# timlawrenz/DINO-X

Measured on AMD Instinct MI355X. Metric: training images/sec (source samples; 2 global views each) ViT-S/16 224px bs256/GPU, higher is better.
Workload: dtype bf16; 1 GPU; ViT-S/16 224x224x3 2.5D slice stacks, scale-aware, 2 views/sample, DINO+Gram loss, AdamW+EMA; per_gpu_batch=256, global_batch=256, local_crops=0, out_dim=8192, parallelism=dp1, hipgraph=False

## Files before the change

### dino-x_amd/csrc/gemm_bf16_areg.hip

```cpp
#include "common.h"
#include "kernels.h"
#include <type_traits>

namespace dinox {

typedef __attribute__((address_space(3))) void ar_lds_void;
typedef __attribute__((address_space(1))) const void ar_gbl_void;
typedef unsigned ar_u32x4 __attribute__((ext_vector_type(4)));

typedef float ar_f32x4 __attribute__((ext_vector_type(4)));

template <bool NT, typename V>
__device__ __forceinline__ void ar_store(char* dst, V v) {
  if (NT) __builtin_nontemporal_store(v, reinterpret_cast<V*>(dst));
  else *reinterpret_cast<V*>(dst) = v;
}

constexpr int AR_BK = 32, AR_BM = 128, AR_BN = 128;
constexpr int AR_SETS = 6;
constexpr int AR_ATILE = AR_BM * AR_BK * 2, AR_BTILE = AR_BN * AR_BK * 2, AR_SLOT = AR_ATILE + AR_BTILE;
constexpr int AR_KBLOCK = 6 * AR_BK * 2;

enum { AR_PLAIN = EPI_ACT_PLAIN, AR_GELU = EPI_ACT_GELU, AR_DGELU = EPI_ACT_DGELU };

__device__ __forceinline__ int ar_xcd_remap(int bid, int nwg) {
  const int q = nwg >> 3, r = nwg & 7, xcd = bid & 7, idx = bid >> 3;
  return (xcd < r ? xcd * (q + 1) : r * (q + 1) + (xcd - r) * q) + idx;
}

template <int OUT_DT, int ACT, bool RES, bool NT>
__global__ __launch_bounds__(256, 3) void gemm_bf16_nt_areg(GemmParams p, int ntiles, int tiles_n) {
  extern __shared__ __attribute__((aligned(16))) char smem[];
  const int lane = threadIdx.x & 63;
  const int wv = __builtin_amdgcn_readfirstlane(threadIdx.x >> 6);
  const int wr = wv >> 1, wc = wv & 1;
  const int tile = ar_xcd_remap(blockIdx.x, ntiles);
  const int tm = tile / tiles_n, tn = tile - tm * tiles_n;
  const int64_t m0 = (int64_t)tm * AR_BM, n0 = (int64_t)tn * AR_BN;
// ... 236 lines not shown
            }
          } else {
#pragma unroll
            for (int u = 0; u < 4; ++u) {
              a[u] = v[u];
              v[u] = gelu_fast(v[u]);
            }
          }
          if (OUT_DT == DINOX_BF16) {
            pa[2 * h] = (unsigned)f32_to_bf16(a[0]) | ((unsigned)f32_to_bf16(a[1]) << 16);
            pa[2 * h + 1] = (unsigned)f32_to_bf16(a[2]) | ((unsigned)f32_to_bf16(a[3]) << 16);
          } else if (p.aux) {
            ar_store<NT>(ablk + ai + 16 * h, ar_f32x4{a[0], a[1], a[2], a[3]});
          }
        }
        if (ACT == AR_DGELU) {
          float x[4];
          if (OUT_DT == DINOX_BF16) {
            const float4 raw = cur_aux[it][0];
            const unsigned w0 = __float_as_uint(h ? raw.z : raw.x), w1 = __float_as_uint(h ? raw.w : raw.y);
            x[0] = __uint_as_float(w0 << 16); x[1] = __uint_as_float(w0 & 0xffff0000u);
            x[2] = __uint_as_float(w1 << 16); x[3] = __uint_as_float(w1 & 0xffff0000u);
          } else {
            const float4 xv = cur_aux[it][h ? AUXV - 1 : 0];
            x[0] = xv.x; x[1] = xv.y; x[2] = xv.z; x[3] = xv.w;
          }
          if (ag) {
#pragma unroll
            for (int u = 0; u < 4; ++u) v[u] *= x[u];
          } else {
// ... 62 lines not shown
```

### dino-x_amd/csrc/gemm_bf16_glds.hip

```cpp

#include "small_common.h"
#include "kernels.h"

namespace dinox {

constexpr int GG_BN = 128;

typedef __attribute__((address_space(3))) void lds_void;
typedef __attribute__((address_space(1))) const void gbl_void;

__device__ __forceinline__ int gg_xcd_remap(int bid, int nwg) {
  const int q = nwg >> 3, r = nwg & 7, xcd = bid & 7, idx = bid >> 3;
  return (xcd < r ? xcd * (q + 1) : r * (q + 1) + (xcd - r) * q) + idx;
}

enum { GG_PLAIN = 0, GG_GELU = 1, GG_DGELU = 2 };

template <int CH>
__device__ __forceinline__ int gg_swz(int row) { return CH == 8 ? ((row >> 1) & 7) : ((row >> 2) & 3); }

template <int OUT_DT, int ACT, bool RES, int GG_BK, int STAGES, int GG_BM>
__global__ __launch_bounds__(256, (GG_BM == 256 ? 2 : (GG_BK == 64 ? 2 : 3))) void gemm_bf16_nt_glds(GemmParams p, int tiles_m, int tiles_n) {
  constexpr int WAVES = 4;
  constexpr int WM = GG_BM / 64;
  constexpr int WROWS = 32 * WM;
  constexpr int A_TILE = GG_BM * GG_BK * 2;
  constexpr int B_TILE = GG_BN * GG_BK * 2;
  constexpr int STAGE_BYTES = A_TILE + B_TILE;
  constexpr int CH = GG_BK / 8;
  constexpr int RPI = 64 / CH;
  constexpr int NQA = GG_BM / RPI / WAVES;
// ... 199 lines not shown
          }
        }
        if (p.aux) {
          const int64_t ai = bz * p.M * p.ldaux + m * p.ldaux + n;
          if (OUT_DT == DINOX_BF16) {
            s16x8 pk;
#pragma unroll
            for (int u = 0; u < 8; ++u) pk[u] = (short)f32_to_bf16(a[u]);
            __builtin_nontemporal_store(pk, reinterpret_cast<s16x8*>((bf16_t*)p.aux + ai));
          } else {
            *reinterpret_cast<float4*>((float*)p.aux + ai) = make_float4(a[0], a[1], a[2], a[3]);
            *reinterpret_cast<float4*>((float*)p.aux + ai + 4) = make_float4(a[4], a[5], a[6], a[7]);
          }
        }
      }
      if (ACT == GG_DGELU) {
        float x[8];
        if (OUT_DT == DINOX_BF16) {
          const float4 raw = cur_aux[it][0];
          const uint32_t w[4] = {__float_as_uint(raw.x), __float_as_uint(raw.y), __float_as_uint(raw.z), __float_as_uint(raw.w)};
#pragma unroll
          for (int u = 0; u < 4; ++u) {
            x[2 * u] = __uint_as_float(w[u] << 16);
            x[2 * u + 1] = __uint_as_float(w[u] & 0xffff0000u);
          }
        } else {
          const float4 x0 = cur_aux[it][0], x1 = cur_aux[it][OUT_DT == DINOX_BF16 ? 0 : 1];
          x[0] = x0.x; x[1] = x0.y; x[2] = x0.z; x[3] = x0.w; x[4] = x1.x; x[5] = x1.y; x[6] = x1.z; x[7] = x1.w;
        }
        if (p.epilogue & DINOX_EPI_AUXGRAD) {
// ... 47 lines not shown
  int bk_auto = p.K <= 512 ? 32 : 64;
  if (bk_auto == 64) {
    const int64_t nt = ceil_div(p.M, (int64_t)128) * ceil_div(p.N, (int64_t)GG_BN) * p.batch;
    const double e512 = (double)nt / (double)(ceil_div(nt, (int64_t)512) * 512), e768 = (double)nt / (double)(ceil_div(nt, (int64_t)768) * 768);
    if (0.9 * e768 > e512) bk_auto = 32;
  }
  const int bk = knob ? knob : bk_auto;
  const int bm = knob_bm ? knob_bm : 128;
  const int stages = bk == 64 ? 2 : 3;

  const int tiles_m = (int)ceil_div(p.M, bm), tiles_n = (int)ceil_div(p.N, GG_BN);
  const int64_t ntile = (int64_t)tiles_m * tiles_n;
  if (ntile > 0x7fffffff) return DINOX_EUNSUPPORTED;
  dim3 grid((unsigned)ntile, (unsigned)p.batch);
  const size_t lds = (size_t)stages * (bm + GG_BN) * bk * 2;
  const int act = (p.epilogue & DINOX_EPI_GELU) ? GG_GELU : (p.epilogue & DINOX_EPI_DGELU) ? GG_DGELU : GG_PLAIN;
  const bool res = (p.epilogue & DINOX_EPI_RESIDUAL) != 0;
  auto launch = [&](auto kern) -> int {
    if (int rc = reserve_lds(reinterpret_cast<const void*>(kern), lds, "gemm_bf16_nt_glds")) return rc;
    hipLaunchKernelGGL(kern, grid, dim3(256), lds, st, p, tiles_m, tiles_n);
    return check_launch("gemm_bf16_nt_glds");
  };
#define GG_K(OUT, ACT, RES, BK, ST, BM) launch(gemm_bf16_nt_glds<OUT, ACT, RES, BK, ST, BM>)
#define GG(OUT, ACT, RES)                                                                               \
  (bm == 256 ? (bk == 32 ? GG_K(OUT, ACT, RES, 32, 3, 256) : GG_K(OUT, ACT, RES, 64, 2, 256))           \
             : (bk == 32 ? GG_K(OUT, ACT, RES, 32, 3, 128) : GG_K(OUT, ACT, RES, 64, 2, 128)))
#define GG_ACT(OUT, RES) (act == GG_GELU ? GG(OUT, GG_GELU, RES) : act == GG_DGELU ? GG(OUT, GG_DGELU, RES) : GG(OUT, GG_PLAIN, RES))
  const int rc = p.out_dtype == DINOX_BF16 ? (res ? GG_ACT(DINOX_BF16, true) : GG_ACT(DINOX_BF16, false))
                                           : (res ? GG_ACT(DINOX_F32, true) : GG_ACT(DINOX_F32, false));
#undef GG_ACT
#undef GG
#undef GG_K
  return rc;
}

}
```

### dino-x_amd/csrc/gemm_pp_common.h

```cpp
#pragma once
#include "common.h"
#include "kernels.h"

namespace dinox {

typedef __attribute__((address_space(3))) void pp_lds_void;
typedef __attribute__((address_space(1))) const void pp_gbl_void;
typedef unsigned pp_u32x4 __attribute__((ext_vector_type(4)));
typedef float pp_f32x4 __attribute__((ext_vector_type(4)));
typedef float pp_f32x2 __attribute__((ext_vector_type(2)));
typedef __bf16 pp_bf16x2 __attribute__((ext_vector_type(2)));

enum { PP_PLAIN = EPI_ACT_PLAIN, PP_GELU = EPI_ACT_GELU, PP_DGELU = EPI_ACT_DGELU };

__device__ __forceinline__ unsigned pp_pack2(float a, float b) {
  const pp_bf16x2 r = __builtin_convertvector(pp_f32x2{a, b}, pp_bf16x2);
  return __builtin_bit_cast(unsigned, r);
}

__device__ __forceinline__ void pp_sync() {
  asm volatile("s_waitcnt lgkmcnt(0)" ::: "memory");
  __builtin_amdgcn_s_barrier();
  __builtin_amdgcn_sched_barrier(0);
}

#define PP_WAIT_BEHIND_STORES(BASE, STEP, sq)                                                                             \
  {                                                                                                                       \
    if ((sq) == 0) asm volatile("s_waitcnt vmcnt(%0)" ::"n"(BASE) : "memory");                                            \
// ... 115 lines not shown
      for (int hh = 0; hh < 2; ++hh) {
        __builtin_amdgcn_sched_barrier(0);
        const pp_f32x4 x4 = hh ? hi : lo;
        float v[4] = {x4[0], x4[1], x4[2], x4[3]}, a[4] = {0.f, 0.f, 0.f, 0.f};
#pragma unroll
        for (int e = 0; e < 4; ++e) v[e] = v[e] * alpha + bias[4 * hh + e];
        if (ACT == PP_GELU) {
#pragma unroll
          for (int e = 0; e < 4; ++e) {
            float y, d;
            gelu_fast_both(v[e], y, d);
            a[e] = d;
            v[e] = y;
          }
        }
        if (ACT == PP_DGELU) {
          float x[4];
          if (OUT_DT == DINOX_BF16) {
            const float4 raw = pf_aux[s % NPF][h][0];
            const unsigned w0 = __float_as_uint(hh ? raw.z : raw.x), w1 = __float_as_uint(hh ? raw.w : raw.y);
            x[0] = __uint_as_float(w0 << 16); x[1] = __uint_as_float(w0 & 0xffff0000u);
            x[2] = __uint_as_float(w1 << 16); x[3] = __uint_as_float(w1 & 0xffff0000u);
          } else {
            const float4 xv = pf_aux[s % NPF][h][hh ? AUXV - 1 : 0];
            x[0] = xv.x; x[1] = xv.y; x[2] = xv.z; x[3] = xv.w;
          }
#pragma unroll
          for (int e = 0; e < 4; ++e) v[e] *= x[e];
        }
        if (RES) {
// ... 82 lines not shown
```

### dino-x_amd/csrc/kernels.h

```cpp
#pragma once
#include <type_traits>

#include "gemm_common.h"
#include "knobs.h"

namespace dinox {

#define GEMM_VARIANTS(X)                                                                                                       \
  X(NtPp, "gemm_bf16_nt_pp") X(NtPp128, "gemm_bf16_nt_pp128") X(NtPp384, "gemm_bf16_nt_pp384") X(NtAreg, "gemm_bf16_nt_areg") \
  X(NtGlds, "gemm_bf16_nt_glds") X(Nt, "gemm_bf16_nt") X(TnBig, "gemm_bf16_tn_big") X(TnDma, "gemm_bf16_tn_dma") X(Tn, "gemm_bf16_tn")
#define X(member, name) member,
enum class GemmVariant { None, GEMM_VARIANTS(X) };
#undef X
#define X(member, name) name,
inline const char* gemm_variant_name(GemmVariant v) {
  static const char* const names[] = {nullptr, GEMM_VARIANTS(X)};
  return names[(int)v];
}
#undef X

int launch_gemm_f32(const GemmParams& p, hipStream_t st);
GemmVariant gemm_bf16_variant(const GemmParams& p);
int launch_gemm_bf16(const GemmParams& p, hipStream_t st);
int64_t gemm_bf16_ws_bytes(const GemmParams& p);
// ... 17 lines not shown
int tn_big_plan(const GemmParams& p, int& tiles_m, int& tiles_n, int& splits, int64_t& kps);
int64_t tn_big_ws_bytes(const GemmParams& p);
int launch_gemm_bf16_tn_big(const GemmParams& p, hipStream_t st, int& splits_out, int& tiles_n_out);

int launch_attention_ref_fwd(const void* qkv, void* o, float* lse, int B, int N, int heads, int d, int dtype, hipStream_t st);
int launch_attention_ref_bwd(const void* d_o, const void* qkv, const void* o, const float* lse, void* dqkv, int B, int N, int heads, int d, int dtype, hipStream_t st);
int launch_attention_bf16_fwd(const void* qkv, void* o, float* lse, int B, int N, int heads, int d, hipStream_t st);
int launch_attention_bf16_bwd(const void* d_o, const void* qkv, const void* o, const float* lse, void* dqkv, float* ws, int B, int N, int heads, int d, hipStream_t st);
bool attention_qkv_fused_ok(int B, int N, int heads, int d, int D);
int launch_attention_qkv_fused_fwd(const void* x, const void* w, const float* bias, void* o, void* qkv_out, float* lse, int B, int N, int heads, int d, int D, hipStream_t st);
int launch_attention_flash_fwd(const void* qkv, void* o, float* lse, int B, int N, int heads, int d, hipStream_t st);
int launch_attention_flash_bwd(const void* d_o, const void* qkv, const void* o, const float* lse, void* dqkv, float* ws, int B, int N, int heads, int d, hipStream_t st);

constexpr int SEG_MAX_CLASSES = 64;

enum { EPI_ACT_PLAIN = 0, EPI_ACT_GELU = 1, EPI_ACT_DGELU = 2 };

template <typename F>
static inline int with_epilogue_case(const GemmParams& p, F&& f) {
  const int act = (p.epilogue & DINOX_EPI_GELU) ? EPI_ACT_GELU : (p.epilogue & DINOX_EPI_DGELU) ? EPI_ACT_DGELU : EPI_ACT_PLAIN;
  const bool res = (p.epilogue & DINOX_EPI_RESIDUAL) != 0;
  auto cases = [&](auto out) -> int {
    switch (act * 2 + (res ? 1 : 0)) {
      case 0: return f(out, std::integral_constant<int, EPI_ACT_PLAIN>{}, std::false_type{});
      case 1: return f(out, std::integral_constant<int, EPI_ACT_PLAIN>{}, std::true_type{});
      case 2: return f(out, std::integral_constant<int, EPI_ACT_GELU>{}, std::false_type{});
      case 4: return f(out, std::integral_constant<int, EPI_ACT_DGELU>{}, std::false_type{});
      default: return DINOX_EUNSUPPORTED;
    }
  };
  return p.out_dtype == DINOX_BF16 ? cases(std::integral_constant<int, DINOX_BF16>{}) : cases(std::integral_constant<int, DINOX_F32>{});
}

struct PersistPlan {
  int tiles_n, units, order, stagger;
  unsigned grid;
};
static inline bool persist_plan(const GemmParams& p, int bm, int bn, int stagger_auto, PersistPlan& pl) {
  const int64_t tiles_n = ceil_div(p.N, (int64_t)bn), units = ceil_div(p.M, (int64_t)bm) * tiles_n;
  if (units > 0x3fffffff) return false;
  const int64_t ncu = device_cu_count();
  pl = {(int)tiles_n, (int)units, knob_int("DINOX_PP_ORDER", 1), knob_int("DINOX_PP_STAGGER", stagger_auto), (unsigned)(units < ncu ? units : ncu)};
// ... 5 lines not shown
```

### dino-x_amd/csrc/optim.hip

```cpp
#include "small_common.h"

namespace dinox {

__global__ __launch_bounds__(256) void adamw_ema_kernel(float* __restrict__ p, const float* __restrict__ g, float* __restrict__ m,
                                                        float* __restrict__ v, float* __restrict__ teacher, int64_t n,
                                                        float lr, float wd, float b1, float b2, float eps, float inv_bc1,
                                                        float inv_sqrt_bc2, float ema, float gscale, float* __restrict__ ws,
                                                        const float* __restrict__ hyper) {
  __shared__ float red[16];
  if (hyper) {
    lr = hyper[0];
    inv_bc1 = hyper[1];
    inv_sqrt_bc2 = hyper[2];
  }
  float sq = 0.f;
  const int64_t n4 = n >> 2;
  const int64_t stride = (int64_t)gridDim.x * blockDim.x;
  for (int64_t i = (int64_t)blockIdx.x * blockDim.x + threadIdx.x; i < n4; i += stride) {
    float4 pp = reinterpret_cast<float4*>(p)[i];
    float4 gg = reinterpret_cast<const float4*>(g)[i];
    float4 mm = reinterpret_cast<float4*>(m)[i];
    float4 vv = reinterpret_cast<float4*>(v)[i];
    float* P = &pp.x; float* G = &gg.x; float* M = &mm.x; float* Vv = &vv.x;
    float4 tt = teacher ? reinterpret_cast<float4*>(teacher)[i] : make_float4(0.f, 0.f, 0.f, 0.f);
// ... 2 lines not shown
    for (int c = 0; c < 4; ++c) {
      const float gr = G[c] * gscale;
      sq += gr * gr;
      float w = P[c] * (1.0f - lr * wd);
      M[c] = b1 * M[c] + (1.0f - b1) * gr;
      Vv[c] = b2 * Vv[c] + (1.0f - b2) * gr * gr;
      const float denom = sqrtf(Vv[c]) * inv_sqrt_bc2 + eps;
      w -= lr * inv_bc1 * (M[c] / denom);
      P[c] = w;
      T[c] = ema * T[c] + (1.0f - ema) * w;
    }
    reinterpret_cast<float4*>(p)[i] = pp;
    reinterpret_cast<float4*>(m)[i] = mm;
    reinterpret_cast<float4*>(v)[i] = vv;
    if (teacher) reinterpret_cast<float4*>(teacher)[i] = tt;
  }
  if (blockIdx.x == 0 && threadIdx.x < (n & 3)) {
    const int64_t i = (n4 << 2) + threadIdx.x;
    const float gr = g[i] * gscale;
    sq += gr * gr;
    float w = p[i] * (1.0f - lr * wd);
    const float mn = b1 * m[i] + (1.0f - b1) * gr, vn = b2 * v[i] + (1.0f - b2) * gr * gr;
    m[i] = mn;
    v[i] = vn;
    w -= lr * inv_bc1 * (mn / (sqrtf(vn) * inv_sqrt_bc2 + eps));
    p[i] = w;
    if (teacher) teacher[i] = ema * teacher[i] + (1.0f - ema) * w;
  }
  sq = block_sum(sq, red);
  if (threadIdx.x == 0) ws[blockIdx.x] = sq;
}

__global__ __launch_bounds__(256) void sumsq_partial(const float* __restrict__ x, int64_t n, float* __restrict__ ws) {
  __shared__ float red[16];
  float a = 0.f;
  for (int64_t i = (int64_t)blockIdx.x * 256 + threadIdx.x; i < n; i += (int64_t)gridDim.x * 256) a += x[i] * x[i];
  a = block_sum(a, red);
  if (threadIdx.x == 0) ws[blockIdx.x] = a;
}

__global__ __launch_bounds__(256) void sum_parts(const float* __restrict__ ws, int n, float* __restrict__ out) {
  __shared__ float red[16];
// ... 51 lines not shown
}

__global__ __launch_bounds__(256) void gelu_fwd_kernel(const float* __restrict__ x, float* __restrict__ y, int64_t n) {
  for (int64_t i = (int64_t)blockIdx.x * 256 + threadIdx.x; i < n; i += (int64_t)gridDim.x * 256) y[i] = gelu_erf(x[i]);
}
__global__ __launch_bounds__(256) void gelu_bwd_kernel(const float* __restrict__ dy, const float* __restrict__ x, float* __restrict__ dx, int64_t n) {
  for (int64_t i = (int64_t)blockIdx.x * 256 + threadIdx.x; i < n; i += (int64_t)gridDim.x * 256) dx[i] = dy[i] * gelu_erf_grad(x[i]);
}

}

using namespace dinox;

static int adamw_launch(float* p, const float* g, float* m, float* v, float* teacher, int64_t n, float lr, float weight_decay,
                        float beta1, float beta2, float eps, float inv_bc1, float inv_sqrt_bc2, float ema, float grad_scale,
                        float* gnorm_sq, float* ws, const float* hyper, void* stream) {
  DX_REQUIRE(p && g && m && v && gnorm_sq && ws, DINOX_EINVAL, "adamw_ema: null pointer");
  DX_REQUIRE(n > 0, DINOX_EINVAL, "adamw_ema: n=%lld", (long long)n);
  DX_REQUIRE(aligned16(p, g, m, v, teacher), DINOX_EALIGN,
             "adamw_ema: arenas must be 16-byte aligned");
  const unsigned blocks = grid_1d(n, 256 * 4, 2048);
  hipStream_t st = as_stream(stream);
  hipLaunchKernelGGL(adamw_ema_kernel, dim3(blocks), dim3(256), 0, st, p, g, m, v, teacher, n, lr, weight_decay, beta1, beta2,
                     eps, inv_bc1, inv_sqrt_bc2, ema, grad_scale, ws, hyper);
  int rc = check_launch("adamw_ema");
  if (rc) return rc;
  hipLaunchKernelGGL(sum_parts, dim3(1), dim3(256), 0, st, ws, (int)blocks, gnorm_sq);
  return check_launch("adamw_ema_norm");
}

extern "C" int dinox_adamw_ema(float* p, const float* g, float* m, float* v, float* teacher, int64_t n, float lr,
                               float weight_decay, float beta1, float beta2, float eps, int step_t, float ema,
                               float grad_scale, float* gnorm_sq, float* ws, void* stream) {
  DX_REQUIRE(step_t >= 1, DINOX_EINVAL, "adamw_ema: step_t=%d", step_t);
  const double bc1 = 1.0 - pow((double)beta1, step_t), bc2 = 1.0 - pow((double)beta2, step_t);
  return adamw_launch(p, g, m, v, teacher, n, lr, weight_decay, beta1, beta2, eps, (float)(1.0 / bc1), (float)(1.0 / sqrt(bc2)), ema,
                      grad_scale, gnorm_sq, ws, nullptr, stream);
}

extern "C" int dinox_adamw_ema_dev(float* p, const float* g, float* m, float* v, float* teacher, int64_t n, const float* hyper,
                                   float weight_decay, float beta1, float beta2, float eps, float ema, float grad_scale,
                                   float* gnorm_sq, float* ws, void* stream) {
  DX_REQUIRE(hyper, DINOX_EINVAL, "adamw_ema_dev: null hyper");
  return adamw_launch(p, g, m, v, teacher, n, 0.f, weight_decay, beta1, beta2, eps, 1.f, 1.f, ema, grad_scale, gnorm_sq, ws, hyper, stream);
}

extern "C" int dinox_sumsq(const float* x, int64_t n, float* out, float* ws, void* stream) {
  DX_REQUIRE(x && out && ws && n > 0, DINOX_EINVAL, "sumsq: bad arguments");
  const unsigned blocks = grid_1d(n, 256 * 8, 2048);
  hipStream_t st = as_stream(stream);
  hipLaunchKernelGGL(sumsq_partial, dim3(blocks), dim3(256), 0, st, x, n, ws);
  hipLaunchKernelGGL(sum_parts, dim3(1), dim3(256), 0, st, ws, (int)blocks, out);
  return check_launch("sumsq");
}

extern "C" int dinox_cast_bf16(const float* src, void* dst, int64_t n, void* stream) {
  DX_REQUIRE(src && dst && n > 0, DINOX_EINVAL, "cast_bf16: bad arguments");
  hipLaunchKernelGGL(cast_bf16_kernel, dim3(grid_1d(n, 256 * 4, 2048)), dim3(256), 0, as_stream(stream), src, (bf16_t*)dst, n);
  return check_launch("cast_bf16");
// ... 31 lines not shown
```

### dino-x_amd/dinox/_lib.py

```python
from __future__ import annotations

import ctypes as C
import os

import torch

_HERE = os.path.dirname(os.path.abspath(__file__))
LIB_PATH = os.environ.get("DINOX_LIB") or os.path.join(_HERE, "libdinox_hip.so")

F32, BF16, U16, I16 = 0, 1, 2, 3
FMT_HU_FLOAT, FMT_HU16_PNG, FMT_WINDOWED_FLOAT = 0, 1, 2
EUNSUPPORTED = -2
EPI_BIAS, EPI_GELU, EPI_DGELU, EPI_RESIDUAL, EPI_ACCUM, EPI_AUXGRAD = 1, 2, 4, 8, 16, 32

vp, i32, i64, f32 = C.c_void_p, C.c_int32, C.c_int64, C.c_float


class GemmArgs(C.Structure):
    _fields_ = [
        ("A", vp), ("B", vp), ("C", vp),
        ("M", i64), ("N", i64), ("K", i64),
        ("lda", i64), ("ldb", i64), ("ldc", i64),
        ("batch", i64), ("strideA", i64), ("strideB", i64), ("strideC", i64),
        ("transA", i32), ("transB", i32), ("in_dtype", i32), ("out_dtype", i32), ("epilogue", i32),
# ... 122 lines not shown
    "dinox_surface3d_stats": (i32, [vp, vp, vp, vp, vp, vp, vp, vp, i64, i32, i32, i32, i32, i32, i32, vp]),
    "dinox_cc_ws_bytes": (i64, [i64, i32, i32, i32]),
    "dinox_cc_label": (i32, [vp, vp, vp, vp, vp, vp, vp, i64, i32, i32, i32, i32, vp]),
    "dinox_cc_filter": (i32, [vp, vp, vp, vp, vp, vp, vp, vp, i64, i32, i32, i32, i32, i32, vp]),
    "dinox_cc_match": (i32, [vp, vp, vp, vp, vp, vp, vp, vp, vp, i64, i32, i32, i32, i32, i32, vp]),
    "dinox_cc3d_ws_bytes": (i64, [i64, i32, i32, i32]),
    "dinox_cc3d_label": (i32, [vp, vp, vp, vp, vp, vp, vp, i64, i32, i32, i32, i32, vp]),
    "dinox_cc3d_filter": (i32, [vp, vp, vp, i32, vp, vp, vp, vp, i64, i32, i32, i32, i32, i32, vp]),
    "dinox_cc3d_match": (i32, [vp, vp, vp, vp, vp, vp, i32, vp, vp, i64, i32, i32, i32, i32, i32, vp]),
    "dinox_attention_rows_ok":(i32, [i32, i32, i32, i32, i32]),
    "dinox_attention_rows": (i32, [vp, vp, vp, vp, i32, i32, i32, i32, i32, i32, vp]),
    "dinox_attention_rollout_step_ok": (i32, [i32, i32, i32, i32]),
    "dinox_attention_rollout_step": (i32, [vp, vp, vp, vp, i32, i32, i32, i32, f32, i32, vp]),
    "dinox_adamw_ema": (i32, [vp, vp, vp, vp, vp, i64, f32, f32, f32, f32, f32, i32, f32, f32, vp, vp, vp]),
    "dinox_adamw_ema_dev": (i32, [vp, vp, vp, vp, vp, i64, vp, f32, f32, f32, f32, f32, f32, vp, vp, vp]),
    "dinox_sumsq": (i32, [vp, i64, vp, vp, vp]),
    "dinox_cast_bf16": (i32, [vp, vp, i64, vp]),
    "dinox_cast_transpose_bf16": (i32, [vp, vp, i32, i32, vp]),
    "dinox_cast_transpose_bf16_multi": (i32, [vp, vp, vp, i32, i64, vp]),
    "dinox_take_rows": (i32, [vp, vp, i64, i64, i32, i64, i32, vp]),
    "dinox_put_rows": (i32, [vp, vp, i64, i64, i32, i64, i32, i32, vp]),
    "dinox_axpy": (i32, [vp, vp, f32, i64, vp]),
    "dinox_lincomb3": (i32, [vp, vp, vp, f32, f32, vp, vp]),
    "dinox_zero": (i32, [vp, i64, vp]),
    "dinox_gelu_fwd": (i32, [vp, vp, i64, vp]),
    "dinox_gelu_bwd": (i32, [vp, vp, vp, i64, vp]),
    "dinox_block_plan": (i32, [i64, i64, i32, i32, i32, i32, i32, i32, C.POINTER(BlockPlan)]),
    "dinox_block_forward": (i32, [C.POINTER(BlockFwdArgs), vp]),
    "dinox_block_backward": (i32, [C.POINTER(BlockBwdArgs), vp]),
    "dinox_retrieval_ws_bytes": (i64, [i64, i64, i64]),
# ... 58 lines not shown
```

### dino-x_amd/dinox/engine.py

```python
from __future__ import annotations

import os
from dataclasses import dataclass
from typing import List, Optional, Tuple

import torch
import torch.distributed as dist

from . import ops
from .dp import GradBucketer, exchanging
from .schedule import get_lr


@dataclass
class StepHyperParams:
    lr: float = 1e-4
    min_lr: float = 1e-6
    warmup_steps: int = 2500
    max_steps: Optional[int] = None
    weight_decay: float = 0.04
    ema: float = 0.996
    teacher_temp: float = 0.04
    student_temp: float = 0.1
    center_momentum: float = 0.9
# ... 198 lines not shown
        return self._step_graph([batch, spacing2b, local_batch, local_spacing])

    def _step_graph(self, inputs: list) -> dict:
        hp = self.hp
        if self._graph is None and self._eager_steps < 2:
            self._eager_steps += 1
            return self._step_eager(*inputs)
        lr = get_lr(self.step_count, hp.max_steps, hp.warmup_steps, hp.lr, hp.min_lr)
        self._hyper_host = torch.tensor(ops.adamw_hyper(lr, hp.beta1, hp.beta2, self.opt_steps + 1), dtype=torch.float32).pin_memory()
        self._hyper_dev.copy_(self._hyper_host, non_blocking=True)
        if self._graph is None:
            self._static = [None if t is None else t.clone() for t in inputs]
            torch.cuda.synchronize()
            self._graph = torch.cuda.CUDAGraph()
            count, opt = self.step_count, self.opt_steps
            with torch.cuda.graph(self._graph):
                self._captured = self._step_eager(*self._static, hyper=self._hyper_dev)
            self.step_count, self.opt_steps = count, opt
        else:
            for dst, src in zip(self._static, inputs):
                if (dst is None) != (src is None) or (dst is not None and dst.shape != src.shape):
                    raise ValueError("use_graph: the batch layout must not change after capture")
                if dst is not None:
                    dst.copy_(src, non_blocking=True)
        self._graph.replay()
        self.step_count += 1
        self.opt_steps += 1
        self.last = dict(self._captured, lr=lr)
        return self.last

    def _step_eager(self, batch, spacing2b=None, local_batch=None, local_spacing=None, mask_noise=None, hyper: Optional[torch.Tensor] = None,
                    patch_mask=None) -> dict:
# ... 30 lines not shown
            bm_work.wait()
            bm.div_(self.world)
        if bm is not None:
            ops.center_ema_(self.center.view(-1), bm, hp.center_momentum)
        if self._ibot_pending is not None:
            sum_count, work = self._ibot_pending
            self._ibot_pending = None
            if work is not None:
                work.wait()
            ops.ibot_center_ema_(self.ibot_center.view(-1), sum_count, hp.center_momentum)
        if self.bucketer is not None:
            self.bucketer.finish()
        self._mark("comm_exposed")
        if last:
            self.opt_steps += 1
            norms = [ops.adamw_ema_(self.flat_p[lo:hi], self.flat_g[lo:hi], self.adam_m[lo:hi], self.adam_v[lo:hi],
                                    None if teacher is None else teacher[lo:hi], lr=lr, weight_decay=hp.weight_decay, beta1=hp.beta1,
                                    beta2=hp.beta2, eps=hp.adam_eps, step_t=self.opt_steps, ema=hp.ema, grad_scale=1.0 / self.world, hyper=hyper)
                     for lo, hi, teacher in self.spans]
            gsq = norms[0]
            ops.weight_cache.clear()
            if self.compute_dtype == torch.bfloat16:
                for sh in self.shadows:
                    sh.refresh()
        else:
            gsq = self._zero1
        self._mark("optimiser_tail")
        self.step_count += 1
        z = self._zero1
        named = {k: (z if v is None else v).detach().reshape(()) for k, v in scalars.items()}
        self.last = {"loss": named.pop("loss"), "dino": named.pop("dino", z.reshape(())), "gram": named.pop("gram", z.reshape(())),
                     "koleo": named.pop("koleo", z.reshape(())), "grad_norm_sq": gsq, "lr": lr, **named}
        return self.last

    def _dino_objective(self, batch, spacing2b, local_batch, local_spacing, mask_noise):
        with ops.compute_dtype(self.compute_dtype), ops.unfold_share():
            main = torch.cuda.current_stream()
# ... 216 lines not shown
```

### dino-x_amd/dinox/ops.py

```python
from __future__ import annotations

import contextlib
import ctypes as C
import math
import operator
import os
import weakref
from typing import NamedTuple, Optional

import numpy as np
import torch

from . import _lib
from ._lib import BF16, EPI_ACCUM, EPI_AUXGRAD, EPI_BIAS, EPI_DGELU, EPI_GELU, EPI_RESIDUAL, F32, BlockBwdArgs, BlockFwdArgs, BlockPlan, GemmArgs, check, lib

Tensor = torch.Tensor
_OVERRIDE: list = []


@contextlib.contextmanager
def compute_dtype(dtype: torch.dtype):
    if dtype not in (torch.float32, torch.bfloat16):
        raise ValueError("compute dtype must be torch.float32 or torch.bfloat16")
    _OVERRIDE.append(dtype)
# ... 266 lines not shown


class ArenaShadow:

    def __init__(self, flat: Tensor, params, offsets) -> None:
        self.flat, self.params, self.offsets = flat, list(params), list(offsets)
        self.index = {p.data_ptr(): i for i, p in enumerate(self.params) if p.numel()}
        self.plain: Optional[Tensor] = None
        self.trans: Optional[Tensor] = None
        self.versions: list = []
        self.wanted: dict = {}
        self.table: Optional[Tensor] = None
        self.table_for: tuple = ()
        self.tiles = 0
        self.served_t: set = set()

    def refresh(self) -> None:
        self.plain = cast_bf16(self.flat, out=self.plain)
        self.versions = [p._version for p in self.params]
        self.served_t = set()
        if self.wanted:
            key = tuple(sorted(self.wanted))
            if key != self.table_for:
                rows, tiles = [], 0
                for i in key:
                    R, Cc = self.wanted[i]
                    rows.append([self.offsets[i], R, Cc, tiles])
                    tiles += ((R + 31) // 32) * ((Cc + 31) // 32)
                self.table = torch.tensor(rows, dtype=torch.int64, device=self.flat.device)
                self.table_for, self.tiles = key, tiles
            if self.trans is None:
                self.trans = torch.empty(self.flat.numel(), dtype=torch.bfloat16, device=self.flat.device)
            check(lib.dinox_cast_transpose_bf16_multi(_p(self.flat), _p(self.trans), _p(self.table), len(self.table_for), self.tiles,
                                                      _stream()), "dinox_cast_transpose_bf16_multi")
# ... 1996 lines not shown
        grad_sink.ready(sw)
        if pb is not None:
            axpy_(sb[1].grad.view(-1), dbt, 1.0)
            grad_sink.ready(sb)
        return None, None
    return dwp[:, :K0].reshape(pw.shape).contiguous(), dbt


def adamw_hyper(lr: float, beta1: float, beta2: float, step_t: int) -> list:
    beta1, beta2 = C.c_float(beta1).value, C.c_float(beta2).value
    return [lr, 1.0 / (1.0 - beta1 ** step_t), 1.0 / math.sqrt(1.0 - beta2 ** step_t)]


def adamw_ema_(p: Tensor, g: Tensor, m: Tensor, v: Tensor, teacher: Optional[Tensor], *, lr: float, weight_decay: float,
               beta1: float, beta2: float, eps: float, step_t: int, ema: float, grad_scale: float = 1.0,
               hyper: Optional[Tensor] = None) -> Tensor:
    _need_cuda(p, g, m, v)
    for t in (p, g, m, v) + ((teacher,) if teacher is not None else ()):
        assert t.is_contiguous() and t.dtype == torch.float32 and t.numel() == p.numel()
    out = torch.empty(1, dtype=torch.float32, device=p.device)
    ws = torch.empty(4096, dtype=torch.float32, device=p.device)
    if hyper is not None:
        assert hyper.is_cuda and hyper.dtype == torch.float32 and hyper.numel() == 3
        check(lib.dinox_adamw_ema_dev(_p(p), _p(g), _p(m), _p(v), _p(teacher), p.numel(), _p(hyper), weight_decay, beta1, beta2, eps, ema,
                                      grad_scale, _p(out), _p(ws), _stream()), "dinox_adamw_ema_dev")
        return out
    check(lib.dinox_adamw_ema(_p(p), _p(g), _p(m), _p(v), _p(teacher), p.numel(), lr, weight_decay, beta1, beta2, eps, step_t, ema,
                              grad_scale, _p(out), _p(ws), _stream()), "dinox_adamw_ema")
    return out


def sumsq(x: Tensor) -> Tensor:
    x = _c(x)
    out = torch.empty(1, dtype=torch.float32, device=x.device)
    ws = torch.empty(4096, dtype=torch.float32, device=x.device)
    check(lib.dinox_sumsq(_p(x), x.numel(), _p(out), _p(ws), _stream()), "dinox_sumsq")
# ... 1015 lines not shown
```

### include/dinox.h

```cpp
#ifndef DINOX_H
#define DINOX_H

#include <stddef.h>
#include <stdint.h>

#ifdef __cplusplus
extern "C" {
#endif

#define DINOX_ABI_VERSION 3

#define DINOX_F32 0
#define DINOX_BF16 1
#define DINOX_U16 2
#define DINOX_I16 3

#define DINOX_OK 0
#define DINOX_EINVAL (-1)
#define DINOX_EUNSUPPORTED (-2)
#define DINOX_EALIGN (-3)

int dinox_version(void);
const char* dinox_last_error(void);
int dinox_device_ok(void);
// ... 157 lines not shown
int dinox_attention_rows_ok(int B, int N, int heads, int d, int Q);
int dinox_attention_rows(const void* qkv, const int* query_idx, float* probs, float* lse, int B, int N, int heads, int d, int Q, int dtype,
                         void* stream);

int dinox_attention_rollout_step_ok(int B, int N, int heads, int d);
size_t dinox_attention_rollout_step_ws_bytes(int B, int N, int heads);
int dinox_attention_rollout_step(const void* qkv, const float* w_in, float* w_out, void* ws, int B, int N, int heads, int d, float residual,
                                 int dtype, void* stream);

int dinox_adamw_ema(float* p, const float* g, float* m, float* v, float* teacher, int64_t n, float lr,
                    float weight_decay, float beta1, float beta2, float eps, int step_t, float ema,
                    float grad_scale, float* gnorm_sq, float* ws, void* stream);
int dinox_adamw_ema_dev(float* p, const float* g, float* m, float* v, float* teacher, int64_t n, const float* hyper,
                        float weight_decay, float beta1, float beta2, float eps, float ema, float grad_scale,
                        float* gnorm_sq, float* ws, void* stream);
int dinox_sumsq(const float* x, int64_t n, float* out, float* ws, void* stream);
int dinox_cast_bf16(const float* src, void* dst, int64_t n, void* stream);
int dinox_cast_transpose_bf16(const float* src, void* dst, int R, int C, void* stream);
int dinox_cast_transpose_bf16_multi(const float* src_base, void* dst_base, const int64_t* table, int n_mats,
                                    int64_t total_tiles, void* stream);
int dinox_take_rows(const float* src, void* dst, int64_t V, int64_t src_stride, int D, int64_t dst_row0, int dst_dtype,
                    void* stream);
int dinox_put_rows(const void* src, float* dst, int64_t V, int64_t dst_stride, int D, int64_t src_row0, int src_dtype,
                   int accumulate, void* stream);
int dinox_axpy(float* y, const float* x, float alpha, int64_t n, void* stream);
int dinox_lincomb3(const float* a, const float* b, const float* c, float wb, float wc, float* out, void* stream);
int dinox_zero(void* p, int64_t bytes, void* stream);
int dinox_gelu_fwd(const float* x, float* y, int64_t n, void* stream);
int dinox_gelu_bwd(const float* dy, const float* x, float* dx, int64_t n, void* stream);

// ... 142 lines not shown
```

Baseline: 7583 samples/s.

## Fuse bf16 weight image writes into AdamW and add aux-free GELU epilogue

The AdamW+EMA kernel now also writes bf16 copies of the updated student and teacher weights. The shadow refresh can then skip its separate full cast pass when every span was already filled. A new GELU_ONLY epilogue variant is added for GEMMs with a GELU epilogue but no aux output, which drops the dead aux-store branch. GC is also disabled during graph capture, and the extra image writes add bandwidth to the optimizer kernel.

```diff
diff --git a/dino-x_amd/csrc/gemm_bf16_areg.hip b/dino-x_amd/csrc/gemm_bf16_areg.hip
--- a/dino-x_amd/csrc/gemm_bf16_areg.hip
+++ b/dino-x_amd/csrc/gemm_bf16_areg.hip
@@ -21,7 +21,7 @@
 constexpr int AR_ATILE = AR_BM * AR_BK * 2, AR_BTILE = AR_BN * AR_BK * 2, AR_SLOT = AR_ATILE + AR_BTILE;
 constexpr int AR_KBLOCK = 6 * AR_BK * 2;
 
-enum { AR_PLAIN = EPI_ACT_PLAIN, AR_GELU = EPI_ACT_GELU, AR_DGELU = EPI_ACT_DGELU };
+enum { AR_PLAIN = EPI_ACT_PLAIN, AR_GELU = EPI_ACT_GELU, AR_DGELU = EPI_ACT_DGELU, AR_GELU_ONLY = EPI_ACT_GELU_ONLY };
 
 __device__ __forceinline__ int ar_xcd_remap(int bid, int nwg) {
   const int q = nwg >> 3, r = nwg & 7, xcd = bid & 7, idx = bid >> 3;
@@ -288,6 +288,19 @@
             ar_store<NT>(ablk + ai + 16 * h, ar_f32x4{a[0], a[1], a[2], a[3]});
           }
         }
+        if (ACT == AR_GELU_ONLY) {
+          if (ag) {
+#pragma unroll
+            for (int u = 0; u < 4; ++u) {
+              float y, d;
+              gelu_fast_both(v[u], y, d);
+              v[u] = y;
+            }
+          } else {
+#pragma unroll
+            for (int u = 0; u < 4; ++u) v[u] = gelu_fast(v[u]);
+          }
+        }
         if (ACT == AR_DGELU) {
           float x[4];
           if (OUT_DT == DINOX_BF16) {
diff --git a/dino-x_amd/csrc/gemm_bf16_glds.hip b/dino-x_amd/csrc/gemm_bf16_glds.hip
--- a/dino-x_amd/csrc/gemm_bf16_glds.hip
+++ b/dino-x_amd/csrc/gemm_bf16_glds.hip
@@ -14,7 +14,7 @@
   return (xcd < r ? xcd * (q + 1) : r * (q + 1) + (xcd - r) * q) + idx;
 }
 
-enum { GG_PLAIN = 0, GG_GELU = 1, GG_DGELU = 2 };
+enum { GG_PLAIN = 0, GG_GELU = 1, GG_DGELU = 2, GG_GELU_ONLY = 3 };
 
 template <int CH>
 __device__ __forceinline__ int gg_swz(int row) { return CH == 8 ? ((row >> 1) & 7) : ((row >> 2) & 3); }
@@ -244,6 +244,19 @@
           }
         }
       }
+      if (ACT == GG_GELU_ONLY) {
+        if (p.epilogue & DINOX_EPI_AUXGRAD) {
+#pragma unroll
+          for (int u = 0; u < 8; ++u) {
+            float y, d;
+            gelu_fast_both(v[u], y, d);
+            v[u] = y;
+          }
+        } else {
+#pragma unroll
+          for (int u = 0; u < 8; ++u) v[u] = gelu_fast(v[u]);
+        }
+      }
       if (ACT == GG_DGELU) {
         float x[8];
         if (OUT_DT == DINOX_BF16) {
@@ -321,7 +334,7 @@
   if (ntile > 0x7fffffff) return DINOX_EUNSUPPORTED;
   dim3 grid((unsigned)ntile, (unsigned)p.batch);
   const size_t lds = (size_t)stages * (bm + GG_BN) * bk * 2;
-  const int act = (p.epilogue & DINOX_EPI_GELU) ? GG_GELU : (p.epilogue & DINOX_EPI_DGELU) ? GG_DGELU : GG_PLAIN;
+  const int act = (p.epilogue & DINOX_EPI_GELU) ? (p.aux ? GG_GELU : GG_GELU_ONLY) : (p.epilogue & DINOX_EPI_DGELU) ? GG_DGELU : GG_PLAIN;
   const bool res = (p.epilogue & DINOX_EPI_RESIDUAL) != 0;
   auto launch = [&](auto kern) -> int {
     if (int rc = reserve_lds(reinterpret_cast<const void*>(kern), lds, "gemm_bf16_nt_glds")) return rc;
@@ -332,7 +345,8 @@
 #define GG(OUT, ACT, RES)                                                                               \
   (bm == 256 ? (bk == 32 ? GG_K(OUT, ACT, RES, 32, 3, 256) : GG_K(OUT, ACT, RES, 64, 2, 256))           \
              : (bk == 32 ? GG_K(OUT, ACT, RES, 32, 3, 128) : GG_K(OUT, ACT, RES, 64, 2, 128)))
-#define GG_ACT(OUT, RES) (act == GG_GELU ? GG(OUT, GG_GELU, RES) : act == GG_DGELU ? GG(OUT, GG_DGELU, RES) : GG(OUT, GG_PLAIN, RES))
+#define GG_ACT(OUT, RES) (act == GG_GELU ? GG(OUT, GG_GELU, RES) : act == GG_GELU_ONLY ? GG(OUT, GG_GELU_ONLY, RES) \
+                          : act == GG_DGELU ? GG(OUT, GG_DGELU, RES) : GG(OUT, GG_PLAIN, RES))
   const int rc = p.out_dtype == DINOX_BF16 ? (res ? GG_ACT(DINOX_BF16, true) : GG_ACT(DINOX_BF16, false))
                                            : (res ? GG_ACT(DINOX_F32, true) : GG_ACT(DINOX_F32, false));
 #undef GG_ACT
diff --git a/dino-x_amd/csrc/gemm_pp_common.h b/dino-x_amd/csrc/gemm_pp_common.h
--- a/dino-x_amd/csrc/gemm_pp_common.h
+++ b/dino-x_amd/csrc/gemm_pp_common.h
@@ -11,7 +11,7 @@
 typedef float pp_f32x2 __attribute__((ext_vector_type(2)));
 typedef __bf16 pp_bf16x2 __attribute__((ext_vector_type(2)));
 
-enum { PP_PLAIN = EPI_ACT_PLAIN, PP_GELU = EPI_ACT_GELU, PP_DGELU = EPI_ACT_DGELU };
+enum { PP_PLAIN = EPI_ACT_PLAIN, PP_GELU = EPI_ACT_GELU, PP_DGELU = EPI_ACT_DGELU, PP_GELU_ONLY = EPI_ACT_GELU_ONLY };
 
 __device__ __forceinline__ unsigned pp_pack2(float a, float b) {
   const pp_bf16x2 r = __builtin_convertvector(pp_f32x2{a, b}, pp_bf16x2);
@@ -157,6 +157,14 @@
             v[e] = y;
           }
         }
+        if (ACT == PP_GELU_ONLY) {
+#pragma unroll
+          for (int e = 0; e < 4; ++e) {
+            float y, d;
+            gelu_fast_both(v[e], y, d);
+            v[e] = y;
+          }
+        }
         if (ACT == PP_DGELU) {
           float x[4];
           if (OUT_DT == DINOX_BF16) {
diff --git a/dino-x_amd/csrc/kernels.h b/dino-x_amd/csrc/kernels.h
--- a/dino-x_amd/csrc/kernels.h
+++ b/dino-x_amd/csrc/kernels.h
@@ -55,11 +55,12 @@
 
 constexpr int SEG_MAX_CLASSES = 64;
 
-enum { EPI_ACT_PLAIN = 0, EPI_ACT_GELU = 1, EPI_ACT_DGELU = 2 };
+enum { EPI_ACT_PLAIN = 0, EPI_ACT_GELU = 1, EPI_ACT_DGELU = 2, EPI_ACT_GELU_ONLY = 3 };
 
 template <typename F>
 static inline int with_epilogue_case(const GemmParams& p, F&& f) {
-  const int act = (p.epilogue & DINOX_EPI_GELU) ? EPI_ACT_GELU : (p.epilogue & DINOX_EPI_DGELU) ? EPI_ACT_DGELU : EPI_ACT_PLAIN;
+  const int act = (p.epilogue & DINOX_EPI_GELU) ? (p.aux ? EPI_ACT_GELU : EPI_ACT_GELU_ONLY)
+                  : (p.epilogue & DINOX_EPI_DGELU) ? EPI_ACT_DGELU : EPI_ACT_PLAIN;
   const bool res = (p.epilogue & DINOX_EPI_RESIDUAL) != 0;
   auto cases = [&](auto out) -> int {
     switch (act * 2 + (res ? 1 : 0)) {
@@ -67,6 +68,7 @@
       case 1: return f(out, std::integral_constant<int, EPI_ACT_PLAIN>{}, std::true_type{});
       case 2: return f(out, std::integral_constant<int, EPI_ACT_GELU>{}, std::false_type{});
       case 4: return f(out, std::integral_constant<int, EPI_ACT_DGELU>{}, std::false_type{});
+      case 6: return f(out, std::integral_constant<int, EPI_ACT_GELU_ONLY>{}, std::false_type{});
       default: return DINOX_EUNSUPPORTED;
     }
   };
diff --git a/dino-x_amd/csrc/optim.hip b/dino-x_amd/csrc/optim.hip
--- a/dino-x_amd/csrc/optim.hip
+++ b/dino-x_amd/csrc/optim.hip
@@ -6,7 +6,8 @@
                                                         float* __restrict__ v, float* __restrict__ teacher, int64_t n,
                                                         float lr, float wd, float b1, float b2, float eps, float inv_bc1,
                                                         float inv_sqrt_bc2, float ema, float gscale, float* __restrict__ ws,
-                                                        const float* __restrict__ hyper) {
+                                                        const float* __restrict__ hyper, bf16_t* __restrict__ p_img,
+                                                        bf16_t* __restrict__ t_img) {
   __shared__ float red[16];
   if (hyper) {
     lr = hyper[0];
@@ -40,6 +41,8 @@
     reinterpret_cast<float4*>(m)[i] = mm;
     reinterpret_cast<float4*>(v)[i] = vv;
     if (teacher) reinterpret_cast<float4*>(teacher)[i] = tt;
+    if (p_img) reinterpret_cast<ushort4*>(p_img)[i] = make_ushort4(f32_to_bf16(P[0]), f32_to_bf16(P[1]), f32_to_bf16(P[2]), f32_to_bf16(P[3]));
+    if (t_img) reinterpret_cast<ushort4*>(t_img)[i] = make_ushort4(f32_to_bf16(T[0]), f32_to_bf16(T[1]), f32_to_bf16(T[2]), f32_to_bf16(T[3]));
   }
   if (blockIdx.x == 0 && threadIdx.x < (n & 3)) {
     const int64_t i = (n4 << 2) + threadIdx.x;
@@ -51,7 +54,12 @@
     v[i] = vn;
     w -= lr * inv_bc1 * (mn / (sqrtf(vn) * inv_sqrt_bc2 + eps));
     p[i] = w;
-    if (teacher) teacher[i] = ema * teacher[i] + (1.0f - ema) * w;
+    if (p_img) p_img[i] = f32_to_bf16(w);
+    if (teacher) {
+      const float t = ema * teacher[i] + (1.0f - ema) * w;
+      teacher[i] = t;
+      if (t_img) t_img[i] = f32_to_bf16(t);
+    }
   }
   sq = block_sum(sq, red);
   if (threadIdx.x == 0) ws[blockIdx.x] = sq;
@@ -133,15 +141,17 @@
 
 static int adamw_launch(float* p, const float* g, float* m, float* v, float* teacher, int64_t n, float lr, float weight_decay,
                         float beta1, float beta2, float eps, float inv_bc1, float inv_sqrt_bc2, float ema, float grad_scale,
-                        float* gnorm_sq, float* ws, const float* hyper, void* stream) {
+                        float* gnorm_sq, float* ws, const float* hyper, void* p_img, void* t_img, void* stream) {
   DX_REQUIRE(p && g && m && v && gnorm_sq && ws, DINOX_EINVAL, "adamw_ema: null pointer");
+  DX_REQUIRE(teacher || !t_img, DINOX_EINVAL, "adamw_ema: a teacher image without a teacher");
+  DX_REQUIRE(((uintptr_t)p_img & 7) == 0 && ((uintptr_t)t_img & 7) == 0, DINOX_EALIGN, "adamw_ema: bf16 images must be 8-byte aligned");
   DX_REQUIRE(n > 0, DINOX_EINVAL, "adamw_ema: n=%lld", (long long)n);
   DX_REQUIRE(aligned16(p, g, m, v, teacher), DINOX_EALIGN,
              "adamw_ema: arenas must be 16-byte aligned");
   const unsigned blocks = grid_1d(n, 256 * 4, 2048);
   hipStream_t st = as_stream(stream);
   hipLaunchKernelGGL(adamw_ema_kernel, dim3(blocks), dim3(256), 0, st, p, g, m, v, teacher, n, lr, weight_decay, beta1, beta2,
-                     eps, inv_bc1, inv_sqrt_bc2, ema, grad_scale, ws, hyper);
+                     eps, inv_bc1, inv_sqrt_bc2, ema, grad_scale, ws, hyper, (bf16_t*)p_img, (bf16_t*)t_img);
   int rc = check_launch("adamw_ema");
   if (rc) return rc;
   hipLaunchKernelGGL(sum_parts, dim3(1), dim3(256), 0, st, ws, (int)blocks, gnorm_sq);
@@ -154,14 +164,27 @@
   DX_REQUIRE(step_t >= 1, DINOX_EINVAL, "adamw_ema: step_t=%d", step_t);
   const double bc1 = 1.0 - pow((double)beta1, step_t), bc2 = 1.0 - pow((double)beta2, step_t);
   return adamw_launch(p, g, m, v, teacher, n, lr, weight_decay, beta1, beta2, eps, (float)(1.0 / bc1), (float)(1.0 / sqrt(bc2)), ema,
-                      grad_scale, gnorm_sq, ws, nullptr, stream);
+                      grad_scale, gnorm_sq, ws, nullptr, nullptr, nullptr, stream);
 }
 
 extern "C" int dinox_adamw_ema_dev(float* p, const float* g, float* m, float* v, float* teacher, int64_t n, const float* hyper,
                                    float weight_decay, float beta1, float beta2, float eps, float ema, float grad_scale,
                                    float* gnorm_sq, float* ws, void* stream) {
   DX_REQUIRE(hyper, DINOX_EINVAL, "adamw_ema_dev: null hyper");
-  return adamw_launch(p, g, m, v, teacher, n, 0.f, weight_decay, beta1, beta2, eps, 1.f, 1.f, ema, grad_scale, gnorm_sq, ws, hyper, stream);
+  return adamw_launch(p, g, m, v, teacher, n, 0.f, weight_decay, beta1, beta2, eps, 1.f, 1.f, ema, grad_scale, gnorm_sq, ws, hyper, nullptr, nullptr,
+                      stream);
+}
+
+extern "C" int dinox_adamw_ema_images(float* p, const float* g, float* m, float* v, float* teacher, void* p_img, void* t_img, int64_t n,
+                                      float lr, float weight_decay, float beta1, float beta2, float eps, int step_t, const float* hyper,
+                                      float ema, float grad_scale, float* gnorm_sq, float* ws, void* stream) {
+  if (hyper)
+    return adamw_launch(p, g, m, v, teacher, n, 0.f, weight_decay, beta1, beta2, eps, 1.f, 1.f, ema, grad_scale, gnorm_sq, ws, hyper, p_img, t_img,
+                        stream);
+  DX_REQUIRE(step_t >= 1, DINOX_EINVAL, "adamw_ema_images: step_t=%d", step_t);
+  const double bc1 = 1.0 - pow((double)beta1, step_t), bc2 = 1.0 - pow((double)beta2, step_t);
+  return adamw_launch(p, g, m, v, teacher, n, lr, weight_decay, beta1, beta2, eps, (float)(1.0 / bc1), (float)(1.0 / sqrt(bc2)), ema,
+                      grad_scale, gnorm_sq, ws, nullptr, p_img, t_img, stream);
 }
 
 extern "C" int dinox_sumsq(const float* x, int64_t n, float* out, float* ws, void* stream) {
diff --git a/dino-x_amd/dinox/_lib.py b/dino-x_amd/dinox/_lib.py
--- a/dino-x_amd/dinox/_lib.py
+++ b/dino-x_amd/dinox/_lib.py
@@ -160,6 +160,7 @@
     "dinox_attention_rollout_step": (i32, [vp, vp, vp, vp, i32, i32, i32, i32, f32, i32, vp]),
     "dinox_adamw_ema": (i32, [vp, vp, vp, vp, vp, i64, f32, f32, f32, f32, f32, i32, f32, f32, vp, vp, vp]),
     "dinox_adamw_ema_dev": (i32, [vp, vp, vp, vp, vp, i64, vp, f32, f32, f32, f32, f32, f32, vp, vp, vp]),
+    "dinox_adamw_ema_images": (i32, [vp, vp, vp, vp, vp, vp, vp, i64, f32, f32, f32, f32, f32, i32, vp, f32, f32, vp, vp, vp]),
     "dinox_sumsq": (i32, [vp, i64, vp, vp, vp]),
     "dinox_cast_bf16": (i32, [vp, vp, i64, vp]),
     "dinox_cast_transpose_bf16": (i32, [vp, vp, i32, i32, vp]),
diff --git a/dino-x_amd/dinox/engine.py b/dino-x_amd/dinox/engine.py
--- a/dino-x_amd/dinox/engine.py
+++ b/dino-x_amd/dinox/engine.py
@@ -1,5 +1,6 @@
 from __future__ import annotations
 
+import gc
 import os
 from dataclasses import dataclass
 from typing import List, Optional, Tuple
@@ -236,8 +237,15 @@
             torch.cuda.synchronize()
             self._graph = torch.cuda.CUDAGraph()
             count, opt = self.step_count, self.opt_steps
-            with torch.cuda.graph(self._graph):
-                self._captured = self._step_eager(*self._static, hyper=self._hyper_dev)
+            gc.collect()
+            gc_was_on = gc.isenabled()
+            gc.disable()
+            try:
+                with torch.cuda.graph(self._graph):
+                    self._captured = self._step_eager(*self._static, hyper=self._hyper_dev)
+            finally:
+                if gc_was_on:
+                    gc.enable()
             self.step_count, self.opt_steps = count, opt
         else:
             for dst, src in zip(self._static, inputs):
@@ -298,13 +306,16 @@
         self._mark("comm_exposed")
         if last:
             self.opt_steps += 1
+            lowp = self.compute_dtype == torch.bfloat16
             norms = [ops.adamw_ema_(self.flat_p[lo:hi], self.flat_g[lo:hi], self.adam_m[lo:hi], self.adam_v[lo:hi],
                                     None if teacher is None else teacher[lo:hi], lr=lr, weight_decay=hp.weight_decay, beta1=hp.beta1,
-                                    beta2=hp.beta2, eps=hp.adam_eps, step_t=self.opt_steps, ema=hp.ema, grad_scale=1.0 / self.world, hyper=hyper)
+                                    beta2=hp.beta2, eps=hp.adam_eps, step_t=self.opt_steps, ema=hp.ema, grad_scale=1.0 / self.world, hyper=hyper,
+                                    p_img=self.shadows[0].image(lo, hi) if lowp else None,
+                                    t_img=self.shadows[1].image(lo, hi) if lowp and teacher is not None else None)
                      for lo, hi, teacher in self.spans]
             gsq = norms[0]
             ops.weight_cache.clear()
-            if self.compute_dtype == torch.bfloat16:
+            if lowp:
                 for sh in self.shadows:
                     sh.refresh()
         else:
diff --git a/dino-x_amd/dinox/ops.py b/dino-x_amd/dinox/ops.py
--- a/dino-x_amd/dinox/ops.py
+++ b/dino-x_amd/dinox/ops.py
@@ -304,10 +304,33 @@
         self.table_for: tuple = ()
         self.tiles = 0
         self.served_t: set = set()
+        self.filled: list = []
+
+    def image(self, lo: int, hi: int) -> Tensor:
+        if self.plain is None:
+            self.plain = torch.empty(self.flat.numel(), dtype=torch.bfloat16, device=self.flat.device)
+            self.versions = []
+        self.filled.append((lo, hi))
+        return self.plain[lo:hi]
+
+    def _image_is_current(self, now: list) -> bool:
+        if self.plain is None or not self.filled:
+            return False
+        ends = self.offsets[1:] + [self.flat.numel()]
+        known = len(self.versions) == len(now)
+        for i, (lo, hi) in enumerate(zip(self.offsets, ends)):
+            if lo == hi or any(a <= lo and hi <= b for a, b in self.filled):
+                continue
+            if not (known and self.versions[i] == now[i]):
+                return False
+        return True
 
     def refresh(self) -> None:
-        self.plain = cast_bf16(self.flat, out=self.plain)
-        self.versions = [p._version for p in self.params]
+        now = [p._version for p in self.params]
+        if not self._image_is_current(now):
+            self.plain = cast_bf16(self.flat, out=self.plain)
+        self.filled = []
+        self.versions = now
         self.served_t = set()
         if self.wanted:
             key = tuple(sorted(self.wanted))
@@ -2334,12 +2357,21 @@
 
 def adamw_ema_(p: Tensor, g: Tensor, m: Tensor, v: Tensor, teacher: Optional[Tensor], *, lr: float, weight_decay: float,
                beta1: float, beta2: float, eps: float, step_t: int, ema: float, grad_scale: float = 1.0,
-               hyper: Optional[Tensor] = None) -> Tensor:
+               hyper: Optional[Tensor] = None, p_img: Optional[Tensor] = None, t_img: Optional[Tensor] = None) -> Tensor:
     _need_cuda(p, g, m, v)
     for t in (p, g, m, v) + ((teacher,) if teacher is not None else ()):
         assert t.is_contiguous() and t.dtype == torch.float32 and t.numel() == p.numel()
     out = torch.empty(1, dtype=torch.float32, device=p.device)
     ws = torch.empty(4096, dtype=torch.float32, device=p.device)
+    if p_img is not None or t_img is not None:
+        assert teacher is not None or t_img is None
+        for t in (p_img, t_img):
+            assert t is None or (t.is_cuda and t.is_contiguous() and t.dtype == torch.bfloat16 and t.numel() == p.numel())
+        if hyper is not None:
+            assert hyper.is_cuda and hyper.dtype == torch.float32 and hyper.numel() == 3
+        check(lib.dinox_adamw_ema_images(_p(p), _p(g), _p(m), _p(v), _p(teacher), _p(p_img), _p(t_img), p.numel(), lr, weight_decay, beta1, beta2,
+                                         eps, step_t, _p(hyper), ema, grad_scale, _p(out), _p(ws), _stream()), "dinox_adamw_ema_images")
+        return out
     if hyper is not None:
         assert hyper.is_cuda and hyper.dtype == torch.float32 and hyper.numel() == 3
         check(lib.dinox_adamw_ema_dev(_p(p), _p(g), _p(m), _p(v), _p(teacher), p.numel(), _p(hyper), weight_decay, beta1, beta2, eps, ema,
diff --git a/include/dinox.h b/include/dinox.h
--- a/include/dinox.h
+++ b/include/dinox.h
@@ -195,6 +195,9 @@
 int dinox_adamw_ema_dev(float* p, const float* g, float* m, float* v, float* teacher, int64_t n, const float* hyper,
                         float weight_decay, float beta1, float beta2, float eps, float ema, float grad_scale,
                         float* gnorm_sq, float* ws, void* stream);
+int dinox_adamw_ema_images(float* p, const float* g, float* m, float* v, float* teacher, void* p_img, void* t_img, int64_t n,
+                           float lr, float weight_decay, float beta1, float beta2, float eps, int step_t, const float* hyper,
+                           float ema, float grad_scale, float* gnorm_sq, float* ws, void* stream);
 int dinox_sumsq(const float* x, int64_t n, float* out, float* ws, void* stream);
 int dinox_cast_bf16(const float* src, void* dst, int64_t n, void* stream);
 int dinox_cast_transpose_bf16(const float* src, void* dst, int R, int C, void* stream);
```

Result: no change. 7629 samples/s (median of 6 runs) (+0.6%).
